# ShigemichiMatsuzaki/MSPL

Hardware: AMD Instinct MI355X
Metric: images/sec pseudo-label gen, ESPDNet-UE s=2.0 480x360(->288x480) bs=16 (higher is better)
Workload: dtype f32; 1 GPU; BASELINE configs[1]: ESPDNet-UE s=2.0 C=13 single-source pseudo-label gen (forward + pred+0.5aux argmax + KL uncertainty + histogram), bs=16/GPU, 16x3x288x480 fp32, hipGraph replay, 3 launches in flight per GPU, 2 consecutive batches of 16 per launch; per_gpu_batch=16, batches_in_flight=3, batches_per_launch=2, classes=13

## Files before the change

include/mspl_hip.h:

```cpp
#ifndef MSPL_HIP_H
#define MSPL_HIP_H

#include <stddef.h>
#include <stdint.h>

#ifdef __cplusplus
extern "C" {
#endif

typedef enum {
    MSPL_OK = 0,
    MSPL_ERR_BAD_SHAPE = -1,
    MSPL_ERR_UNSUPPORTED = -2,
    MSPL_ERR_NULL_POINTER = -3,
    MSPL_ERR_HIP = -4
} mspl_status;

typedef struct {
    const float* scale;
    const float* shift;
    const float* alpha;
    const float* pre_add;
    const float* residual;
    const float* reinf_r;
// ... 50 lines not shown
                      int32_t Wo, int32_t align_corners, const mspl_epilogue_t* ep, float* out, void* stream);

int mspl_decoder_merge_fwd(const float* enc, const float* bu, const float* w3, const float* e_scale, const float* e_shift,
                           const float* e_alpha, const float* gate, const float* b_scale, const float* b_shift,
                           const float* b_alpha, const float* wp, const float* p_scale, const float* p_shift,
                           const float* p_alpha, int32_t N, int32_t Cin, int32_t Cout, int32_t P, int32_t H, int32_t W,
                           float* out, void* stream);

int mspl_adaptive_avgpool_fwd(const float* x, int32_t N, int32_t C, int32_t Hi, int32_t Wi,
                              int32_t Ho, int32_t Wo, const mspl_epilogue_t* ep, float* out,
                              void* stream);

int mspl_pointwise_fwd(const float* x, int32_t N, int32_t C, int32_t HW, const mspl_epilogue_t* ep,
                       float* out, void* stream);

int mspl_gap_gate_fwd(const float* x, const float* w, int32_t N, int32_t Cin, int32_t Cout,
                      int32_t HW, float* mean_ws, float* gate, void* stream);

int mspl_fusion_gate_fwd(const float* z, const float* rgb, const float* depth, int64_t count, float* out, void* stream);
int mspl_fusion_gate_bwd(const float* z, const float* rgb, const float* depth, const float* gy, int64_t count,
                         float* gz, float* grgb, float* gdepth, void* stream);

int mspl_avgpool3x3s2_psum_blocks(int32_t H, int32_t W);
int mspl_avgpool3x3s2_psum_fwd(const float* x, int32_t N, int32_t C, int32_t H, int32_t W, const mspl_epilogue_t* ep, float* out,
                               float* psum, void* stream);
int mspl_gate_from_sums_fwd(const float* psum, const float* w, int32_t N, int32_t Cin, int32_t Cout, int32_t nblk, int32_t HW,
                            float* gate, void* stream);

int mspl_down_head_fits(int32_t N, int32_t nin, int32_t n, int32_t groups, int32_t H, int32_t W, uint32_t launch_flags);
int mspl_down_head_psum_blocks(int32_t H, int32_t W);
int mspl_down_head_fwd(const float* x, const float* wp, const float* pscale, const float* pshift, const float* palpha, int32_t N,
                       int32_t nin, int32_t n, int32_t groups, int32_t H, int32_t W, const mspl_epilogue_t* ep, float* r, float* out,
                       float* psum, void* stream);

int64_t mspl_pyr_down_prep_lds_bytes(int32_t N, int32_t P, int32_t h, int32_t w, int32_t nb, const int32_t* hs,
                                     const int32_t* ws);
int mspl_pyr_down_prep_fwd(const float* x, int32_t N, int32_t P, int32_t h, int32_t w, int32_t nb, const int32_t* hs,
                           const int32_t* ws, const float* const* stage_w, float* const* out, void* stream);
int mspl_pyr_down_prep_train_fwd(const float* x, int32_t N, int32_t P, int32_t h, int32_t w, int32_t nb, const int32_t* hs,
                                 const int32_t* ws, const float* const* stage_w, float* const* out, float* const* pooled,
                                 void* stream);
int mspl_pyr_down_mid_bwd(const float* const* g_e, const float* const* pooled, const float* const* stage_w, int32_t N, int32_t P,
                          int32_t h, int32_t w, int32_t nb, const int32_t* hs, const int32_t* ws, float* const* gw,
                          float* const* gx, void* stream);

int mspl_pyrpool_fused_fwd(const float* x, int32_t N, int32_t P, int32_t h, int32_t w, int32_t nb,
                           const int32_t* hs, const int32_t* ws, const float* const* stage_w,
                           const float* const* down_e, const float* br_scale, const float* br_shift,
                           const float* br_alpha, const float* merge_w, const mspl_epilogue_t* ep,
                           float* out, void* stream);

int mspl_pyrpool_fused_train_fwd(const float* x, int32_t N, int32_t P, int32_t h, int32_t w, int32_t nb,
                                 const int32_t* hs, const int32_t* ws, const float* const* stage_w,
                                 const float* const* down_e, const float* br_scale, const float* br_shift,
                                 const float* br_alpha, const float* merge_w, const mspl_epilogue_t* ep,
                                 float* out, float* zcat, void* stream);
int mspl_pyrpool_fused_train_fits(int32_t N, int32_t P, int32_t h, int32_t w, int32_t nb, const int32_t* hs, const int32_t* ws);
int mspl_pyrpool_merge_bwd(const float* gy, const float* mraw, const float* zcat, int32_t N, int32_t P, int32_t h,
                           int32_t w, int32_t nb, const float* br_scale, const float* br_shift, const float* br_alpha,
                           const float* br_mean, const float* br_inv, const float* merge_w, const float* m_scale,
                           const float* m_shift, const float* m_alpha, const float* m_mean, const float* m_inv,
                           float* gt, float* g_br_scale, float* g_br_shift, float* g_br_alpha, float* g_merge_w,
                           float* g_m_scale, float* g_m_shift, float* g_m_alpha, void* stream);
int mspl_pyrpool_branch_bwd_fits(int32_t N, int32_t P, int32_t h, int32_t w, int32_t nb, const int32_t* hs, const int32_t* ws);
int mspl_pyrpool_branch_bwd(const float* x, int32_t N, int32_t P, int32_t h, int32_t w, int32_t nb, const int32_t* hs,
                            const int32_t* ws, const float* const* stage_w, const float* const* gt, float* const* gw,
// ... 212 lines not shown
```

mspl_amd/_native.py:

```python
import ctypes
import os

import torch

_HERE = os.path.dirname(os.path.abspath(__file__))
LIB_PATH = os.environ.get('MSPL_HIP_LIB') or os.path.join(_HERE, 'lib', 'libmspl_hip.so')

c_f32p = ctypes.c_void_p
c_i32 = ctypes.c_int32
c_i64 = ctypes.c_int64


class Epilogue(ctypes.Structure):
    _fields_ = [('scale', ctypes.c_void_p), ('shift', ctypes.c_void_p), ('alpha', ctypes.c_void_p),
                ('pre_add', ctypes.c_void_p), ('residual', ctypes.c_void_p), ('reinf_r', ctypes.c_void_p),
                ('reinf_w', ctypes.c_void_p), ('gate', ctypes.c_void_p),
                ('out_ctot', c_i32), ('out_coff', c_i32), ('raw_out', ctypes.c_void_p),
                ('struct_size', ctypes.c_uint32), ('flags', ctypes.c_uint32)]


class TrainRec(ctypes.Structure):
    _fields_ = [(n, ctypes.c_void_p) for n in ('scale_x', 'scale_y', 'dscale_x', 'dscale_y', 'out_x', 'out_y', 'near_x', 'near_y',
                                               'near_out_x', 'near_out_y')] + \
               [(n, c_i32) for n in ('sh', 'sw', 'pad_h', 'pad_w', 'crop_i', 'crop_j', 'flip', 'reserved')]
# ... 5 lines not shown
ABI_VERSION = 4
ERR_UNSUPPORTED = -2
LAUNCH_THROUGHPUT = 1
LAUNCH_K2_STREAM_OFF = 2
LAUNCH_K2_STREAM_FORCE = 4


_EP = ctypes.POINTER(Epilogue)

SIGNATURES = {
    'mspl_eesp_dw_hff_fwd': [c_f32p, c_f32p, ctypes.POINTER(c_i32), c_i32, c_i32, c_i32, c_i32, c_i32, _EP,
                             c_f32p, ctypes.c_void_p],
    'mspl_eesp_proj_dw_hff_fits': [c_i32] * 6 + [ctypes.POINTER(c_i32), ctypes.c_uint32],
    'mspl_eesp_proj_dw_hff_fwd': [c_f32p] * 6 + [ctypes.POINTER(c_i32)] + [c_i32] * 6 + [_EP, c_f32p, ctypes.c_void_p],
    'mspl_eesp_dw_exp_fits': [c_i32] * 4 + [ctypes.POINTER(c_i32), ctypes.c_uint32],
    'mspl_eesp_dw_exp_pack_floats': [c_i32],
    'mspl_eesp_dw_exp_pack': [c_f32p] * 5 + [c_i32] * 3 + [ctypes.POINTER(c_i32), c_f32p, ctypes.c_void_p],
    'mspl_eesp_dw_exp_fwd': [c_f32p, c_f32p, ctypes.POINTER(c_i32)] + [c_i32] * 4 + [_EP, c_f32p, ctypes.c_void_p],
    'mspl_eesp_dw_exp_next_pack_floats': [c_i32],
    'mspl_eesp_dw_exp_next_pack': [c_f32p, c_i32, c_f32p, ctypes.c_void_p],
    'mspl_eesp_dw_exp_next_fwd': [c_f32p, c_f32p, ctypes.POINTER(c_i32)] + [c_i32] * 4 + [_EP, c_f32p] + [c_f32p] * 5 + [ctypes.c_void_p],
    'mspl_conv1x1_fwd': [c_f32p, c_f32p, c_i32, c_i32, c_i32, c_i32, c_i32, _EP, c_f32p, ctypes.c_void_p],
    'mspl_conv3x3_fwd': [c_f32p, c_f32p, c_i32, c_i32, c_i32, c_i32, c_i32, c_i32, c_i32, c_i32, _EP, c_f32p,
                         ctypes.c_void_p],
    'mspl_avgpool3x3s2_fwd': [c_f32p, c_i32, c_i32, c_i32, c_i32, _EP, c_f32p, ctypes.c_void_p],
    'mspl_bilinear_fwd': [c_f32p, c_i32, c_i32, c_i32, c_i32, c_i32, c_i32, c_i32, _EP, c_f32p, ctypes.c_void_p],
    'mspl_decoder_merge_fwd': [c_f32p] * 14 + [c_i32] * 6 + [c_f32p, ctypes.c_void_p],
    'mspl_adaptive_avgpool_fwd': [c_f32p, c_i32, c_i32, c_i32, c_i32, c_i32, c_i32, _EP, c_f32p, ctypes.c_void_p],
    'mspl_avgpool3x3s2_psum_fwd': [c_f32p, c_i32, c_i32, c_i32, c_i32, _EP, c_f32p, c_f32p, ctypes.c_void_p],
    'mspl_avgpool3x3s2_psum_blocks': [c_i32, c_i32],
    'mspl_down_head_fits': [c_i32] * 6 + [ctypes.c_uint32],
    'mspl_down_head_psum_blocks': [c_i32, c_i32],
    'mspl_down_head_fwd': [c_f32p] * 5 + [c_i32] * 6 + [_EP, c_f32p, c_f32p, c_f32p, ctypes.c_void_p],
    'mspl_gate_from_sums_fwd': [c_f32p, c_f32p, c_i32, c_i32, c_i32, c_i32, c_i32, c_f32p, ctypes.c_void_p],
    'mspl_pointwise_fwd': [c_f32p, c_i32, c_i32, c_i32, _EP, c_f32p, ctypes.c_void_p],
    'mspl_gap_gate_fwd': [c_f32p, c_f32p, c_i32, c_i32, c_i32, c_i32, c_f32p, c_f32p, ctypes.c_void_p],
    'mspl_fusion_gate_fwd': [c_f32p, c_f32p, c_f32p, c_i64, c_f32p, ctypes.c_void_p],
    'mspl_fusion_gate_bwd': [c_f32p, c_f32p, c_f32p, c_f32p, c_i64, c_f32p, c_f32p, c_f32p, ctypes.c_void_p],
    'mspl_pyrpool_fused_fwd': [c_f32p, c_i32, c_i32, c_i32, c_i32, c_i32, ctypes.POINTER(c_i32), ctypes.POINTER(c_i32),
                               ctypes.POINTER(ctypes.c_void_p), ctypes.POINTER(ctypes.c_void_p), c_f32p, c_f32p, c_f32p,
                               c_f32p, _EP, c_f32p, ctypes.c_void_p],
    'mspl_pyrpool_fused_train_fwd': [c_f32p, c_i32, c_i32, c_i32, c_i32, c_i32, ctypes.POINTER(c_i32), ctypes.POINTER(c_i32),
                                     ctypes.POINTER(ctypes.c_void_p), ctypes.POINTER(ctypes.c_void_p), c_f32p, c_f32p, c_f32p,
                                     c_f32p, _EP, c_f32p, c_f32p, ctypes.c_void_p],
    'mspl_pyrpool_fused_train_fits': [c_i32] * 5 + [ctypes.POINTER(c_i32), ctypes.POINTER(c_i32)],
    'mspl_pyrpool_merge_bwd': [c_f32p] * 3 + [c_i32] * 5 + [c_f32p] * 19 + [ctypes.c_void_p],
    'mspl_pyrpool_branch_bwd_fits': [c_i32] * 5 + [ctypes.POINTER(c_i32), ctypes.POINTER(c_i32)],
    'mspl_pyrpool_branch_bwd': [c_f32p] + [c_i32] * 5 + [ctypes.POINTER(c_i32), ctypes.POINTER(c_i32)] +
                               [ctypes.POINTER(ctypes.c_void_p)] * 3 + [c_f32p, c_f32p, c_f32p, ctypes.c_void_p],
    'mspl_label_epilogue_fwd': [c_f32p, c_f32p, c_i32, c_i32, c_i32, c_i32, c_i32, c_i32, c_i32, c_i32,
                                ctypes.c_void_p, ctypes.c_void_p, c_f32p, c_f32p, c_f32p, c_f32p, ctypes.c_void_p],
    'mspl_label_epilogue_hist_fwd': [c_f32p, c_f32p, c_i32, c_i32, c_i32, c_i32, c_i32, c_i32, c_i32, c_i32,
                                     ctypes.c_void_p, ctypes.c_void_p, c_f32p, ctypes.c_void_p, c_i32, ctypes.c_void_p, c_i64,
                                     ctypes.c_void_p],
    'mspl_label_epilogue_hist_workspace_bytes': [c_i32, c_i32, c_i32],
    'mspl_label_epilogue_hist_fits': [c_i32] * 8,
    'mspl_conv_bwd_data': [c_f32p, c_f32p] + [c_i32] * 10 + [c_f32p, ctypes.c_void_p],
    'mspl_conv_bwd_weight': [c_f32p, c_f32p] + [c_i32] * 10 + [c_f32p, ctypes.c_void_p],
    'mspl_affine_prelu_bwd': [c_f32p] * 7 + [c_i32] * 3 + [c_f32p] * 5 + [ctypes.c_void_p],
    'mspl_bn_train_small_fits': [c_i32] * 3,
    'mspl_bn_train_small_fwd': [c_f32p] * 5 + [c_i32] * 3 + [ctypes.c_float] * 2 + [c_f32p] * 2 + [ctypes.c_void_p] + [c_f32p] * 5 + [ctypes.c_void_p],
    'mspl_bn_train_small_bwd': [c_f32p] * 9 + [c_i32] * 4 + [c_f32p] * 5 + [ctypes.c_void_p],
    'mspl_bn_train_prelu_bwd_apply': [c_f32p] * 7 + [c_i32] * 3 + [c_f32p, ctypes.c_void_p],
    'mspl_pyrpool_merge_fwd': [c_f32p] + [c_i32] * 5 + [c_f32p] * 5 + [ctypes.c_void_p],
    'mspl_bn_stats_path_add': [c_f32p] * 4 + [c_i32] * 4 + [ctypes.c_void_p],
    'mspl_bn_fused_workspace_bytes': [c_i32],
# ... 64 lines not shown
                           [c_f32p] * 12 + [ctypes.c_void_p],
    'mspl_eesp_dw_bwd': [c_f32p, c_f32p, c_f32p, ctypes.POINTER(c_i32), c_i32, c_i32, c_i32, c_i32, c_i32, c_f32p,
                         ctypes.POINTER(ctypes.c_void_p), ctypes.c_void_p],
    'mspl_png_writer_create': [c_i32, c_i32],
    'mspl_png_writer_submit': [ctypes.c_void_p, ctypes.c_void_p, c_i32, c_i32, c_i32, ctypes.POINTER(ctypes.c_char_p), ctypes.c_void_p],
    'mspl_png_writer_poll': [ctypes.c_void_p, c_i64, c_i32],
    'mspl_png_writer_destroy': [ctypes.c_void_p],
    'mspl_abi_version': [],
    'mspl_sum_n': [ctypes.POINTER(ctypes.c_void_p), c_i32, c_i64, c_f32p, ctypes.c_void_p],
    'mspl_sum_n_planes': [ctypes.POINTER(ctypes.c_void_p), c_i32, c_f32p, ctypes.c_float, c_i32, c_i32, c_f32p, ctypes.c_void_p],
    'mspl_transpose_weights': [ctypes.c_void_p, ctypes.c_void_p, c_i32, ctypes.c_void_p],
    'mspl_adam_step': [c_f32p, c_f32p, c_f32p, c_f32p, c_i64, ctypes.c_float, ctypes.c_double, ctypes.c_double, ctypes.c_float, ctypes.c_float,
                       c_i32, ctypes.c_void_p],
    'mspl_merge_labels_fwd': [ctypes.POINTER(ctypes.c_void_p), c_i32, c_i64, c_i32, c_i32, c_i32, ctypes.c_void_p,
                              ctypes.c_void_p, ctypes.c_void_p],
}


def _load():
    if not os.path.isfile(LIB_PATH):
        raise ImportError(
            'mspl_amd: %s not found. Build it with `python -c "import __graft_entry__ as g; g.build()"` or '
            '`make -C mspl_amd/csrc` (hipcc --offload-arch=gfx950). There is no CPU fallback.' % LIB_PATH)
    lib = ctypes.CDLL(LIB_PATH)
    for name, argtypes in SIGNATURES.items():
        fn = getattr(lib, name)
        fn.argtypes = argtypes
        fn.restype = ctypes.c_int
    lib.mspl_pyr_down_prep_lds_bytes.restype = ctypes.c_int64
    lib.mspl_nid_workspace_floats.restype = ctypes.c_int64
    lib.mspl_eesp_dw_exp_pack_floats.restype = ctypes.c_int64
    lib.mspl_bn_fused_workspace_bytes.restype = ctypes.c_int64
    lib.mspl_eesp_dw_exp_next_pack_floats.restype = ctypes.c_int64
    lib.mspl_label_epilogue_hist_workspace_bytes.restype = ctypes.c_int64
    lib.mspl_train_transform_workspace_bytes.restype = ctypes.c_int64
    lib.mspl_png_writer_create.restype = ctypes.c_void_p
    lib.mspl_png_writer_submit.restype = ctypes.c_int64
    lib.mspl_version.restype = ctypes.c_char_p
    if lib.mspl_abi_version() != ABI_VERSION:
        raise ImportError('mspl_amd: %s has ABI revision %d, this package binds revision %d: rebuild the library (make -C mspl_amd/csrc)'
                          % (LIB_PATH, lib.mspl_abi_version(), ABI_VERSION))
    lib.mspl_last_error.argtypes = [ctypes.c_char_p, ctypes.c_size_t]
    lib.mspl_last_error.restype = ctypes.c_size_t
    return lib


lib = _load()


def last_error():
    buf = ctypes.create_string_buffer(512)
    lib.mspl_last_error(buf, 512)
    return buf.value.decode()


def check(status):
    if status != 0:
        raise RuntimeError('mspl_hip (%d): %s' % (status, last_error()))


def version():
    return lib.mspl_version().decode()
```

mspl_amd/layers.py:

```python
import math
import os
import weakref

import torch
from torch import nn

from . import autograd as ag
from . import ops
from .ops import Epi

config_inp_reinf = 3
PYR_SCALES = (2.0, 1.5, 1.0, 0.5, 0.1)


_PARAM_EPOCH = [0]


def bump_param_epoch():
    _PARAM_EPOCH[0] += 1


def _key(tensors):
    return (_PARAM_EPOCH[0],) + tuple((t.data_ptr(), t._version) for t in tensors)

# ... 102 lines not shown
    for t in outs:
        t.record_stream(cur)


def _training_path():
    return torch.is_grad_enabled()


def _conv_train(x, conv):
    if conv.kernel_size[0] == 3 and conv.dilation[0] != 1:
        raise RuntimeError('mspl_amd: dilated 3x3 convolutions only occur inside EESP (fused branch op)')
    return ag.conv(x, conv.weight, conv.stride[0], conv.groups)


def _bn_act(z, bn, alpha=None, pre_add=None, residual=None):
    if bn.training:
        if pre_add is not None:
            z, pre_add = z + pre_add, None
        if _FUSED_BN_TRAIN:
            return ag.bn_train_prelu(z, bn, alpha, residual)
        scale, shift = ag.bn_batch_stats(z, bn)
    else:
        scale, shift = train_fold(bn)
        return ag.bn_prelu(z, bn, scale, shift, alpha, pre_add=pre_add, residual=residual)
    return ag.affine_prelu(z, scale, shift, alpha, pre_add=pre_add, residual=residual)


_FUSED_TRAIN_FWD = os.environ.get('MSPL_TRAIN_FUSED_FWD', '1') != '0'
_EESP_DW_BN = os.environ.get('MSPL_EESP_DW_BN', '1') != '0'
_CONV_SKIP = os.environ.get('MSPL_CONV_SKIP', '1') != '0'
_FUSED_BN_TRAIN = os.environ.get('MSPL_FUSED_BN_TRAIN', '1') != '0'
_FUSED_DW_EXP = os.environ.get('MSPL_EESP_EXP', '1') != '0'
_FUSED_DOWN_HEAD = os.environ.get('MSPL_DOWN_HEAD', '1') != '0'
_FUSED_DEC_MERGE = True
_FUSED_NEXT_PROJ = os.environ.get('MSPL_EESP_NEXT', '1') != '0'
_FUSED_EESP_TRAIN = os.environ.get('MSPL_FUSED_EESP_TRAIN', '1') != '0'
_FUSED_PYR_TRAIN = os.environ.get('MSPL_FUSED_PYR_TRAIN', '1') != '0'


def _conv_bn_act(x, conv, bn, alpha=None, pre_add=None, residual=None):
    if bn.training or not _FUSED_TRAIN_FWD:
        return _bn_act(_conv_train(x, conv), bn, alpha, pre_add, residual)
    if conv.kernel_size[0] == 3 and conv.dilation[0] != 1:
        raise RuntimeError('mspl_amd: dilated 3x3 convolutions only occur inside EESP (fused branch op)')
    scale, shift = train_fold(bn)
    return ag.conv_bn_prelu(x, conv.weight, conv.stride[0], conv.groups, bn, scale, shift, alpha, pre_add, residual)


def train_fold(bn):
    def build():
        scale = bn.weight * ag.frozen_bn_inv(bn)
        return scale, torch.addcmul(bn.bias, bn.running_mean, scale, value=-1.0)
    return cached(bn, 'tfold', [bn.weight, bn.bias, bn.running_mean, bn.running_var], build)


def prefold_frozen_bn(model):
    bns = [m for m in model.modules() if isinstance(m, nn.BatchNorm2d) and not m.training]
    if not bns:
        return
    with torch.no_grad():
        invs = [ag.frozen_bn_inv(m) for m in bns]
        scales = torch._foreach_mul([m.weight for m in bns], invs)
        shifts = torch._foreach_addcmul([m.bias for m in bns], [m.running_mean for m in bns], scales, value=-1.0)
    for m, sc, sh in zip(bns, scales, shifts):
        store = m.__dict__.setdefault('_mspl_cache', {})
        store['tfold'] = (_key([m.weight, m.bias, m.running_mean, m.running_var]), (sc, sh))
# ... 129 lines not shown

class EESP(nn.Module):
    def __init__(self, nIn, nOut, stride=1, k=4, r_lim=7, down_method='esp'):
        super().__init__()
        self.stride = stride
        n = int(nOut / k)
        n1 = nOut - (k - 1) * n
        assert down_method in ['avg', 'esp'], 'One of these is suppported (avg or esp)'
        assert n == n1, "n(={}) and n1(={}) should be equal for Depth-wise Convolution ".format(n, n1)
        if k != 4:
            raise NotImplementedError('mspl_amd: the fused EESP kernel is built for k=4 branches')
        self.proj_1x1 = CBR(nIn, n, 1, stride=1, groups=k)
        self.dilations = eesp_dilations(r_lim, k)
        self.spp_dw = nn.ModuleList(CDilated(n, n, kSize=3, stride=stride, groups=n, d=d) for d in self.dilations)
        self.conv_1x1_exp = CB(nOut, nOut, 1, 1, groups=k)
        self.br_after_cat = BR(nOut)
        self.module_act = nn.PReLU(nOut)
        self.downAvg = True if down_method == 'avg' else False
        self.k = k

    def _dw_weights(self):
        ws = [m.conv.weight for m in self.spp_dw]
        return cached(self, 'w4', ws, lambda: torch.stack([w.reshape(-1, 3, 3) for w in ws]).contiguous())

    def _dw_exp_packed(self, H, W):
        br, exp = self.br_after_cat, self.conv_1x1_exp
        deps = [m.conv.weight for m in self.spp_dw] + [br.bn.weight, br.bn.bias, br.bn.running_mean, br.bn.running_var,
                                                      br.act.weight, exp.conv.weight]

        def build():
            bs, bb = bn_fold(br.bn)
            return ops.eesp_dw_exp_pack(self._dw_weights(), bs, bb, br.act.weight, exp.conv.weight, H, W, self.dilations)
        return cached(self, 'dwexp%dx%d' % (H, W), deps, build)

    def reduce_transform(self, input):
        scale, shift = bn_fold(self.br_after_cat.bn)
        pj = self.proj_1x1
        if ops.eesp_proj_dw_hff_fits(input.shape, pj.conv.out_channels, pj.conv.groups, self.dilations, self.stride):
            ps, pb = bn_fold(pj.bn)
            return ops.eesp_proj_dw_hff(input, pj.conv.weight, ps, pb, pj.act.weight, self._dw_weights(), self.dilations,
                                        pj.conv.groups, Epi(scale, shift, self.br_after_cat.act.weight))
        return self.transform(pj(input))

    def transform(self, o1):
        scale, shift = bn_fold(self.br_after_cat.bn)
        return ops.eesp_dw_hff(o1, self._dw_weights(), self.dilations, self.stride,
                               Epi(scale, shift, self.br_after_cat.act.weight))

    def _forward_train(self, input):
        pj, br, exp = self.proj_1x1, self.br_after_cat, self.conv_1x1_exp
        if _FUSED_EESP_TRAIN and not (pj.bn.training or br.bn.training or exp.bn.training):
            strided_avg = self.stride == 2 and self.downAvg
            residual = (not strided_avg) and self.stride == 1 and exp.conv.out_channels == input.shape[1]
            cfg = {'stride': self.stride, 'dil': tuple(self.dilations), 'groups': pj.conv.groups, 'residual': residual}
            ws = [m.conv.weight for m in self.spp_dw]
            folds = [ag.frozen_bn_fold(bn, *train_fold(bn)) for bn in (pj.bn, br.bn, exp.bn)]
            return ag.EESPFn.apply(input, cfg, *folds, pj.conv.weight, pj.bn.weight, pj.bn.bias,
                                   pj.act.weight, ws[0], ws[1], ws[2], ws[3], br.bn.weight, br.bn.bias, br.act.weight,
                                   exp.conv.weight, exp.bn.weight, exp.bn.bias, None if strided_avg else self.module_act.weight)
        has_res = self.stride == 1 and exp.conv.out_channels == input.shape[1] and not (self.stride == 2 and self.downAvg)
        skip = input
        if has_res and pj.bn.training and _CONV_SKIP and input.requires_grad:
            z1, skip = ag.conv_skip(input, pj.conv.weight, pj.conv.groups)
            o1 = _bn_act(z1, pj.bn, pj.act.weight)
        else:
            o1 = self.proj_1x1(input)
# ... 107 lines not shown
                shift = shift + rb
            return scale.contiguous(), shift.contiguous(), rw
        return cached(self, 'epi%d' % int(with_reinf), deps, build)

    def _forward_train(self, input, input2, alias=None):
        avg_out = ag.avgpool(input)
        eesp_out = self.eesp(input if alias is None else alias)
        reinf = None
        if input2 is not None:
            with torch.no_grad():
                pyr = input2 if isinstance(input2, ImagePyramid) else ImagePyramid(input2)
                img = pyr.at_height(avg_out.shape[2])
            if img.shape[3] != avg_out.shape[3]:
                raise RuntimeError('The size of tensor a (%d) must match the size of tensor b (%d) at non-singleton '
                                   'dimension 3' % (avg_out.shape[3], img.shape[3]))
            reinf = self.inp_reinf(img)
        return ag.down_tail(avg_out, eesp_out, self.act.weight, reinf)

    def forward(self, input, input2=None, _alias=None):
        if _training_path():
            return self._forward_train(input, input2, _alias)
        N, _, H, W = input.shape
        Ho, Wo = (H - 1) // 2 + 1, (W - 1) // 2 + 1
        out = torch.empty((N, self.nout, Ho, Wo), device=input.device, dtype=torch.float32)
        r = None
        if input2 is not None:
            pyr = input2 if isinstance(input2, ImagePyramid) else ImagePyramid(input2)
            with fork(0, (pyr.levels[0],)):
                r = self.inp_reinf[0](pyr.at_height(Ho))
            if r.shape[3] != Wo:
                raise RuntimeError('The size of tensor a (%d) must match the size of tensor b (%d) at non-singleton '
                                   'dimension 3' % (Wo, r.shape[3]))
        pj = self.eesp.proj_1x1
        if _FUSED_DOWN_HEAD and ops.down_head_fits(input.shape, pj.conv.out_channels, pj.conv.groups):
            join(0, (r,))
            scale, shift, rw = self._epilogue_vectors(r is not None)
            ep = Epi(scale, shift, self.act.weight, reinf_r=r, reinf_w=rw)
            ps, pb = bn_fold(pj.bn)
            o1, sums = ops.down_head(input, pj.conv.weight, ps, pb, pj.act.weight, pj.conv.groups, ep, out)
            _remember_plane_sums(input, sums)
            cat = self.eesp.transform(o1)
            ops.conv1x1(cat, self.eesp.conv_1x1_exp.conv.weight, self.eesp.k, ep, out=(out, self.nin))
            return out
        cat = self.eesp.reduce_transform(input)
        join(0, (r,))
        scale, shift, rw = self._epilogue_vectors(r is not None)
        ep = Epi(scale, shift, self.act.weight, reinf_r=r, reinf_w=rw)
        _, sums = ops.avgpool3x3s2(input, ep, out=(out, 0), plane_sums=True)
        _remember_plane_sums(input, sums)
        ops.conv1x1(cat, self.eesp.conv_1x1_exp.conv.weight, self.eesp.k, ep, out=(out, self.nin))
        return out


_PLANE_SUMS = weakref.WeakKeyDictionary()


class _TensorKey(object):
    __slots__ = ('__weakref__',)


def _remember_plane_sums(t, sums):
    key = getattr(t, '_mspl_key', None)
    if key is None:
        key = _TensorKey()
        t._mspl_key = key
    _PLANE_SUMS[key] = (t.data_ptr(), t._version, sums)


def _recall_plane_sums(t):
    key = getattr(t, '_mspl_key', None)
    hit = _PLANE_SUMS.get(key) if key is not None else None
    if hit is None or hit[0] != t.data_ptr() or hit[1] != t._version:
        return None
    return hit[2]

# ... 204 lines not shown
```

mspl_amd/ops.py:

```python
import ctypes
import math

import torch

from . import _native as nat
from ._native import Epilogue, check, lib


def _stream():
    return ctypes.c_void_p(torch.cuda.current_stream().cuda_stream)


def _f32(t, name):
    if not isinstance(t, torch.Tensor) or not t.is_cuda:
        raise RuntimeError('mspl_amd: %s must be a CUDA (ROCm) tensor; there is no CPU path' % name)
    if t.dtype != torch.float32:
        raise RuntimeError('mspl_amd: %s must be float32, got %s' % (name, t.dtype))
    if not t.is_contiguous():
        t = t.contiguous()
    return t


def _p(t):
    return None if t is None else ctypes.c_void_p(t.data_ptr())
# ... 233 lines not shown
        return dst
    nblk = lib.mspl_avgpool3x3s2_psum_blocks(H, W)
    if nblk <= 0:
        check(nblk)
    sums = torch.empty((N * C, nblk), device=x.device, dtype=torch.float32)
    check(lib.mspl_avgpool3x3s2_psum_fwd(_p(x), N, C, H, W, ctypes.byref(s), _p(dst), _p(sums), _stream()))
    return dst, sums


def down_head_fits(shape, n, groups):
    N, nin, H, W = [int(v) for v in shape]
    return bool(lib.mspl_down_head_fits(N, nin, int(n), int(groups), H, W, current_launch_flags()))


def down_head(x, wproj, pscale, pshift, palpha, groups, ep, out):
    x, wproj = _f32(x, 'x'), _f32(wproj, 'projection weight')
    N, nin, H, W = x.shape
    n = wproj.shape[0]
    if wproj.numel() != n * (nin // groups) or nin % groups or n % groups:
        raise RuntimeError('mspl_amd: down_head weight %s does not match nin=%d groups=%d' % (tuple(wproj.shape), nin, groups))
    ps, pb, pa = _vec(pscale, n, 'pscale'), _vec(pshift, n, 'pshift'), _vec(palpha, n, 'palpha')
    dst, coff = _dest((out, 0), (N, nin, H // 2, W // 2), x)
    s, keep = _build(ep, dst, coff, N, nin, (H // 2) * (W // 2))
    nblk = lib.mspl_down_head_psum_blocks(H, W)
    if nblk <= 0:
        check(nblk)
    r = torch.empty((N, n, H, W), device=x.device, dtype=torch.float32)
    sums = torch.empty((N * nin, nblk), device=x.device, dtype=torch.float32)
    check(lib.mspl_down_head_fwd(_p(x), _p(wproj), _p(ps), _p(pb), _p(pa), N, nin, n, int(groups), H, W, ctypes.byref(s), _p(r),
                                 _p(dst), _p(sums), _stream()))
    return r, sums


def gate_from_sums(plane_sums, w, hw):
    w = _f32(w, 'w')
    Cout = w.shape[0]
    Cin = w.numel() // Cout
    planes, nblk = plane_sums.shape
    N = planes // Cin
    if planes != N * Cin or plane_sums.dtype != torch.float32 or not plane_sums.is_contiguous():
        raise RuntimeError('mspl_amd: gate_from_sums: sums %s do not match Cin=%d' % (tuple(plane_sums.shape), Cin))
    gate = torch.empty((N, Cout), device=w.device, dtype=torch.float32)
    check(lib.mspl_gate_from_sums_fwd(_p(plane_sums), _p(w), N, Cin, Cout, nblk, int(hw), _p(gate), _stream()))
    return gate


def decoder_merge_shape_ok(Cin, Cout, P, H, W):
    groups = math.gcd(Cin, Cout)
    cg, cob = Cin // groups, Cout // groups
    if H % 2 or W % 2 or H < 2 or W < 2 or P not in (2, 6, 10, 16) or Cout > 1024:
        return False
    return (cg, cob) in ((1, 1), (8, 3)) or ((cg, cob) == (4, 1) and groups >= 16 and W % 4 == 0 and 16 <= W <= 256 and H >= 4)


def decoder_merge(enc, bu, w3, e_epi, gate, b_epi, wp, p_epi):
    enc, bu, w3, wp = _f32(enc, 'enc'), _f32(bu, 'bu'), _f32(w3, 'w3'), _f32(wp, 'wp')
    N, Cin, H, W = enc.shape
    Cout, P = w3.shape[0], wp.shape[0]
    if tuple(bu.shape) != (N, Cout, H // 2, W // 2) or H % 2 or W % 2:
        return None
    groups = math.gcd(Cin, Cout)
    if tuple(w3.shape) != (Cout, Cin // groups, 3, 3) or wp.numel() != P * Cout:
        raise RuntimeError('mspl_amd: decoder_merge weights %s / %s do not match Cin=%d Cout=%d'
                           % (tuple(w3.shape), tuple(wp.shape), Cin, Cout))
    gate = _vec(gate, N * Cout, 'gate')
    es, eb, ea = [_vec(t, Cout, 'expansion epilogue') for t in e_epi]
# ... 228 lines not shown
```

Baseline: 21390 images/s.

## Fuse strided dilated depthwise, HFF, BN-PReLU and grouped 1x1 expansion in downsampling EESP

Adds a HIP kernel for the strided EESP downsampling block. It computes the four stride-2 dilated depthwise branches with hierarchical feature fusion and BN+PReLU in LDS, then runs the grouped 1x1 expansion on MFMA 32x32x2 f32. The outer epilogue with reinforcement is applied directly into the concatenated output. This removes the intermediate concat tensor round-trip and separate launches, in exchange for a shape-specialised path (n=32, W=120, dilations 1-4) plus a packed-weight cache.

```diff
diff --git a/include/mspl_hip.h b/include/mspl_hip.h
--- a/include/mspl_hip.h
+++ b/include/mspl_hip.h
@@ -106,6 +106,13 @@
 int mspl_down_head_fwd(const float* x, const float* wp, const float* pscale, const float* pshift, const float* palpha, int32_t N,
                        int32_t nin, int32_t n, int32_t groups, int32_t H, int32_t W, const mspl_epilogue_t* ep, float* r, float* out,
                        float* psum, void* stream);
+
+int mspl_down_dw_exp_fits(int32_t N, int32_t n, int32_t H, int32_t W, const int32_t dil[4], uint32_t launch_flags);
+int64_t mspl_down_dw_exp_pack_floats(int32_t n);
+int mspl_down_dw_exp_pack(const float* w4, const float* bscale, const float* bshift, const float* balpha, const float* wexp,
+                          int32_t n, float* packed, void* stream);
+int mspl_down_dw_exp_fwd(const float* r, const float* packed, const int32_t dil[4], int32_t N, int32_t n, int32_t H, int32_t W,
+                         const mspl_epilogue_t* ep, float* out, void* stream);
 
 int64_t mspl_pyr_down_prep_lds_bytes(int32_t N, int32_t P, int32_t h, int32_t w, int32_t nb, const int32_t* hs,
                                      const int32_t* ws);
diff --git a/mspl_amd/_native.py b/mspl_amd/_native.py
--- a/mspl_amd/_native.py
+++ b/mspl_amd/_native.py
@@ -61,6 +61,10 @@
     'mspl_down_head_fits': [c_i32] * 6 + [ctypes.c_uint32],
     'mspl_down_head_psum_blocks': [c_i32, c_i32],
     'mspl_down_head_fwd': [c_f32p] * 5 + [c_i32] * 6 + [_EP, c_f32p, c_f32p, c_f32p, ctypes.c_void_p],
+    'mspl_down_dw_exp_fits': [c_i32] * 4 + [ctypes.POINTER(c_i32), ctypes.c_uint32],
+    'mspl_down_dw_exp_pack_floats': [c_i32],
+    'mspl_down_dw_exp_pack': [c_f32p] * 5 + [c_i32, c_f32p, ctypes.c_void_p],
+    'mspl_down_dw_exp_fwd': [c_f32p, c_f32p, ctypes.POINTER(c_i32)] + [c_i32] * 4 + [_EP, c_f32p, ctypes.c_void_p],
     'mspl_gate_from_sums_fwd': [c_f32p, c_f32p, c_i32, c_i32, c_i32, c_i32, c_i32, c_f32p, ctypes.c_void_p],
     'mspl_pointwise_fwd': [c_f32p, c_i32, c_i32, c_i32, _EP, c_f32p, ctypes.c_void_p],
     'mspl_gap_gate_fwd': [c_f32p, c_f32p, c_i32, c_i32, c_i32, c_i32, c_f32p, c_f32p, ctypes.c_void_p],
@@ -191,6 +195,7 @@
     lib.mspl_eesp_dw_exp_pack_floats.restype = ctypes.c_int64
     lib.mspl_bn_fused_workspace_bytes.restype = ctypes.c_int64
     lib.mspl_eesp_dw_exp_next_pack_floats.restype = ctypes.c_int64
+    lib.mspl_down_dw_exp_pack_floats.restype = ctypes.c_int64
     lib.mspl_label_epilogue_hist_workspace_bytes.restype = ctypes.c_int64
     lib.mspl_train_transform_workspace_bytes.restype = ctypes.c_int64
     lib.mspl_png_writer_create.restype = ctypes.c_void_p
diff --git a/mspl_amd/csrc/down_dw_exp.hip b/mspl_amd/csrc/down_dw_exp.hip
--- /dev/null
+++ b/mspl_amd/csrc/down_dw_exp.hip
@@ -0,0 +1,303 @@
+#include <stdlib.h>
+
+#include "common.hpp"
+
+namespace mspl {
+
+typedef float dx_f32x16 __attribute__((ext_vector_type(16)));
+
+constexpr int DX_REC = 48;
+constexpr int DX_MAXD = 4;
+
+__device__ __forceinline__ int dx_xcd_remap(int bid, int nwg) {
+    const int q = nwg >> 3, r = nwg & 7, xcd = bid & 7;
+    const int base = (xcd < r) ? xcd * (q + 1) : r * (q + 1) + (xcd - r) * q;
+    return base + (bid >> 3);
+}
+
+__global__ void down_dw_exp_pack_kernel(const float* __restrict__ w4, const float* __restrict__ bscale, const float* __restrict__ bshift,
+                                        const float* __restrict__ balpha, const float* __restrict__ wexp, int n,
+                                        float* __restrict__ dwp, float* __restrict__ ap) {
+    const int i = blockIdx.x * blockDim.x + threadIdx.x;
+    if (i < n * DX_REC) {
+        const int c = i / DX_REC, f = i - c * DX_REC;
+        const int k = f / 12, e = f - k * 12;
+        float v;
+        if (e < 9) v = w4[((size_t)k * n + c) * 9 + e];
+        else if (e == 9) v = bscale[k * n + c];
+        else if (e == 10) v = bshift[k * n + c];
+        else v = balpha[k * n + c];
+        dwp[i] = v;
+    }
+    const int hk = n / 2;
+    if (i < 4 * 64 * hk) {
+        const int lane = i & 63, s = (i >> 6) % hk, g = i / (hk * 64);
+        const int m = lane & 31, k = 2 * s + (lane >> 5);
+        ap[i] = m < n ? wexp[(size_t)(g * n + m) * n + k] : 0.f;
+    }
+}
+
+template <int NCH, int WO, int TH, int KC>
+__global__ __launch_bounds__(512, 4) void down_dw_exp_kernel(const float* __restrict__ r, const float* __restrict__ dwp,
+                                                             const float* __restrict__ ap, Epi e, float* __restrict__ out,
+                                                             int H, int bands, int nwg) {
+    constexpr int MAXD = DX_MAXD;
+    constexpr int ROWS = 2 * TH - 1 + 2 * MAXD;
+    constexpr int PH = 2;
+    constexpr int HS = WO + 2 * PH;
+    constexpr int RS = 2 * HS;
+    constexpr int PX = TH * WO;
+    constexpr int NS64 = (PX + 63) / 64;
+    constexpr int SPW = NS64 / 2;
+    constexpr int SLOTS = NS64 * 64;
+    constexpr int NCHUNK = NCH / KC;
+    constexpr int LPR = WO <= 64 ? 64 : 128;
+    constexpr int RPP = 512 / LPR;
+    constexpr int IPT = (KC * ROWS + RPP - 1) / RPP;
+    static_assert(WO <= 128, "staging: one float2 column per thread");
+    constexpr int TPW = KC * NS64 / 8;
+    static_assert(NS64 % 2 == 0 && (KC * NS64) % 8 == 0, "eight waves: (group, half of the sub-tiles) / (channel, sub-tile)");
+    static_assert(KC % 2 == 0 && NCH % KC == 0 && NCHUNK >= 2 && NCH % 8 == 0 && NCH <= 32, "chunking");
+    static_assert(WO % 2 == 0, "8-byte stores: pixel pairs never straddle a row");
+
+    constexpr int RT_F = KC * ROWS * RS, BB_F = 4 * KC * SLOTS;
+    static_assert((2 * RT_F + 2 * BB_F) * 4 <= 64 * 1024, "static LDS");
+    __shared__ __attribute__((aligned(16))) float lds_[2 * RT_F + 2 * BB_F];
+    float* const rt_[2] = {lds_, lds_ + RT_F};
+    float* const bb_[2] = {lds_ + 2 * RT_F, lds_ + 2 * RT_F + BB_F};
+
+    const int tid = threadIdx.x;
+    const int lane = tid & 63;
+    const int wave = __builtin_amdgcn_readfirstlane(tid >> 6);
+    const int li = lane & 31, half = lane >> 5;
+
+    const int lid = dx_xcd_remap(blockIdx.x, nwg);
+    const int band = lid % bands;
+    const int img = lid / bands;
+    const int y0 = band * TH;
+    const int Ho = H >> 1;
+    const int HWi = H * 2 * WO;
+
+    const float* rimg = r + (size_t)img * NCH * HWi;
+    const int c2 = tid % LPR, r0 = tid / LPR;
+    const bool cok = c2 < WO;
+    float2 sv[IPT];
+    auto load_chunk = [&](int c) {
+        const float* rc = rimg + (size_t)c * KC * HWi + 2 * (cok ? c2 : 0);
+#pragma unroll
+        for (int q = 0; q < IPT; ++q) {
+            const int fr = r0 + RPP * q;
+            const int j = fr / ROWS, row = fr - j * ROWS;
+            const int gy = 2 * y0 - MAXD + row;
+            const bool ok = cok && fr < KC * ROWS && gy >= 0 && gy < H;
+            const float2 v = *reinterpret_cast<const float2*>(rc + (ok ? j * HWi + gy * (2 * WO) : 0));
+            sv[q] = ok ? v : make_float2(0.f, 0.f);
+        }
+    };
+    auto store_chunk = [&](float* dst) {
+        float* d = dst + r0 * RS + PH + c2;
+#pragma unroll
+        for (int q = 0; q < IPT; ++q) {
+            if (cok && r0 + RPP * q < KC * ROWS) {
+                d[RPP * q * RS] = sv[q].x;
+                d[RPP * q * RS + HS] = sv[q].y;
+            }
+        }
+    };
+
+    auto dw_stage = [&](int c, const float* src, float* dst) {
+#pragma unroll
+        for (int u = 0; u < TPW; ++u) {
+            const int task = wave + 8 * u;
+            const int j = task % KC, st = task / KC;
+            const float* rec = dwp + (size_t)(c * KC + j) * DX_REC;
+            float wv[DX_REC];
+#pragma unroll
+            for (int i = 0; i < DX_REC; ++i) wv[i] = rec[i];
+            const int p = 64 * st + lane;
+            const int pc = p < PX ? p : PX - 1;
+            const int ty = (TH > 1) ? pc / WO : 0;
+            const int tx = pc - ty * WO;
+            const float* tp = src + j * (ROWS * RS) + (2 * ty + MAXD) * RS + PH + tx;
+            float prev = 0.f;
+            float tap[4][9];
+#pragma unroll
+            for (int k = 0; k < 4; ++k) {
+                const int d = k + 1;
+#pragma unroll
+                for (int ky = 0; ky < 3; ++ky)
+#pragma unroll
+                    for (int kx = 0; kx < 3; ++kx) {
+                        const int q = ky * 3 + kx;
+                        const int o = (kx - 1) * d;
+                        const int col = (o & 1) ? HS + (o - 1) / 2 : o / 2;
+                        if (q == 4 && k > 0) tap[k][q] = tap[0][4];
+                        else tap[k][q] = tp[(ky - 1) * d * RS + col];
+                    }
+                float a = 0.f;
+#pragma unroll
+                for (int ky = 0; ky < 3; ++ky) {
+                    a = fmaf(wv[k * 12 + ky * 3 + 0], tap[k][ky * 3 + 0], a);
+                    a = fmaf(wv[k * 12 + ky * 3 + 1], tap[k][ky * 3 + 1], a);
+                    a = fmaf(wv[k * 12 + ky * 3 + 2], tap[k][ky * 3 + 2], a);
+                }
+                a += prev;
+                prev = a;
+                float q = fmaf(a, wv[k * 12 + 9], wv[k * 12 + 10]);
+                q = q > 0.f ? q : wv[k * 12 + 11] * q;
+                dst[(k * KC + j) * SLOTS + p] = q;
+            }
+        }
+    };
+
+    const int g = wave & 3, sh = wave >> 2;
+    dx_f32x16 acc[SPW][2];
+#pragma unroll
+    for (int u = 0; u < SPW; ++u)
+#pragma unroll
+        for (int i = 0; i < 16; ++i) { acc[u][0][i] = 0.f; acc[u][1][i] = 0.f; }
+    const float* apw = ap + (size_t)g * (NCH / 2) * 64 + lane;
+    float a_cur[KC / 2], a_nxt[KC / 2];
+    auto load_a = [&](int c, float (&dst)[KC / 2]) {
+#pragma unroll
+        for (int i = 0; i < KC / 2; ++i) dst[i] = apw[(c * (KC / 2) + i) * 64];
+    };
+    auto mm_stage = [&](const float* src, const float (&av)[KC / 2]) {
+#pragma unroll
+        for (int u = 0; u < SPW; ++u) {
+            const float* bp = src + (g * KC + half) * SLOTS + 64 * (sh * SPW + u) + 2 * li;
+#pragma unroll
+            for (int i = 0; i < KC / 2; ++i) {
+                const float2 b2 = *reinterpret_cast<const float2*>(bp + 2 * i * SLOTS);
+                acc[u][0] = __builtin_amdgcn_mfma_f32_32x32x2f32(av[i], b2.x, acc[u][0], 0, 0, 0);
+                acc[u][1] = __builtin_amdgcn_mfma_f32_32x32x2f32(av[i], b2.y, acc[u][1], 0, 0, 0);
+            }
+        }
+    };
+
+    load_chunk(0);
+    load_a(0, a_cur);
+    for (int i = tid; i < 2 * KC * ROWS * 8; i += 512) {
+        const int c8 = i & 7, k4 = c8 & 3;
+        const int rr = i >> 3;
+        lds_[rr * RS + (c8 >> 2) * HS + (k4 < 2 ? k4 : WO + k4)] = 0.f;
+    }
+    store_chunk(rt_[0]);
+    load_chunk(1);
+    __syncthreads();
+    dw_stage(0, rt_[0], bb_[0]);
+    store_chunk(rt_[1]);
+    __syncthreads();
+
+#pragma unroll
+    for (int c = 0; c < NCHUNK; ++c) {
+        if (c + 2 < NCHUNK) load_chunk(c + 2);
+        if (c + 1 < NCHUNK) {
+            if ((c & 1) == 0) load_a(c + 1, a_nxt); else load_a(c + 1, a_cur);
+            dw_stage(c + 1, rt_[(c + 1) & 1], bb_[(c + 1) & 1]);
+        }
+        if ((c & 1) == 0) mm_stage(bb_[c & 1], a_cur); else mm_stage(bb_[c & 1], a_nxt);
+        if (c + 2 < NCHUNK) store_chunk(rt_[c & 1]);
+        if (c + 1 < NCHUNK) __syncthreads();
+    }
+
+    const int rows_here = (Ho - y0) < TH ? (Ho - y0) : TH;
+    const int npx = rows_here * WO;
+#pragma unroll
+    for (int u = 0; u < SPW; ++u) {
+        const int p = 64 * (sh * SPW + u) + 2 * li;
+        const bool pok = p < npx;
+        const int pix = y0 * WO + (pok ? p : 0);
+        float2 r0 = make_float2(0.f, 0.f), r1 = r0, r2 = r0;
+        if (e.reinf_r) {
+            const float* rp = e.reinf_r + (size_t)img * 3 * e.hw + pix;
+            r0 = *reinterpret_cast<const float2*>(rp);
+            r1 = *reinterpret_cast<const float2*>(rp + e.hw);
+            r2 = *reinterpret_cast<const float2*>(rp + 2 * (size_t)e.hw);
+        }
+#pragma unroll
+        for (int rg = 0; rg < 4; ++rg) {
+            if (8 * rg + 8 > NCH) continue;
+#pragma unroll
+            for (int q = 0; q < 4; ++q) {
+                const int rr = rg * 4 + q;
+                const int cabs = e.coff + g * NCH + 8 * rg + 4 * half + q;
+                const EpiCh ch = epi_channel(e, cabs);
+                float v0 = fmaf(acc[u][0][rr], ch.scale, ch.shift);
+                float v1 = fmaf(acc[u][1][rr], ch.scale, ch.shift);
+                if (e.reinf_r) {
+                    v0 += ch.rw0 * r0.x + ch.rw1 * r1.x + ch.rw2 * r2.x;
+                    v1 += ch.rw0 * r0.y + ch.rw1 * r1.y + ch.rw2 * r2.y;
+                }
+                v0 = v0 > 0.f ? v0 : ch.alpha * v0;
+                v1 = v1 > 0.f ? v1 : ch.alpha * v1;
+                if (pok) store_out2(out + epi_offset(e, img, cabs, pix), make_float2(v0, v1));
+            }
+            asm volatile("" ::: "memory");
+        }
+    }
+}
+
+static int dx_plan(int n, int H, int W, const int32_t* dil) {
+    if (!dil || H < 2 || (H & 1)) return 0;
+    if (!(dil[0] == 1 && dil[1] == 2 && dil[2] == 3 && dil[3] == 4)) return 0;
+    if (n == 32 && W == 120) return 2;
+    return 0;
+}
+
+}
+
+using namespace mspl;
+
+extern "C" int mspl_down_dw_exp_fits(int32_t N, int32_t n, int32_t H, int32_t W, const int32_t dil[4], uint32_t flags) {
+    static const int enabled = MSPL_TUNE_INT("MSPL_DOWN_DW_EXP", 1);
+    (void)flags;
+    if (!enabled || N < 1) return 0;
+    return dx_plan(n, H, W, dil) != 0 ? 1 : 0;
+}
+
+extern "C" int64_t mspl_down_dw_exp_pack_floats(int32_t n) { return (int64_t)n * DX_REC + 4ll * 64 * (n / 2); }
+
+extern "C" int mspl_down_dw_exp_pack(const float* w4, const float* bscale, const float* bshift, const float* balpha,
+                                     const float* wexp, int32_t n, float* packed, void* stream_) {
+    hipStream_t stream = static_cast<hipStream_t>(stream_);
+    MSPL_REQUIRE(w4 && bscale && bshift && balpha && wexp && packed, MSPL_ERR_NULL_POINTER, "down_dw_exp_pack: null pointer");
+    MSPL_REQUIRE(n == 32, MSPL_ERR_UNSUPPORTED, "down_dw_exp_pack: n=%d not covered", n);
+    const int total = 4 * 64 * (n / 2);
+    hipLaunchKernelGGL(down_dw_exp_pack_kernel, dim3((unsigned)ceil_div(total, 256)), dim3(256), 0, stream, w4, bscale, bshift, balpha,
+                       wexp, n, packed, packed + (size_t)n * DX_REC);
+    MSPL_CHECK_LAUNCH("down_dw_exp_pack");
+    return MSPL_OK;
+}
+
+extern "C" int mspl_down_dw_exp_fwd(const float* r, const float* packed, const int32_t dil[4], int32_t N, int32_t n, int32_t H,
+                                    int32_t W, const mspl_epilogue_t* ep, float* out, void* stream_) {
+    hipStream_t stream = static_cast<hipStream_t>(stream_);
+    MSPL_REQUIRE(r && packed && dil && ep && out, MSPL_ERR_NULL_POINTER, "down_dw_exp: null pointer");
+    MSPL_REQUIRE(N >= 1 && H >= 1 && W >= 1, MSPL_ERR_BAD_SHAPE, "down_dw_exp: N=%d H=%d W=%d", N, H, W);
+    if (int rc = check_epi(ep, 4 * n, "down_dw_exp")) return rc;
+    MSPL_REQUIRE(ep->scale && ep->shift && ep->alpha, MSPL_ERR_NULL_POINTER, "down_dw_exp: the block's epilogue needs scale, shift and alpha");
+    MSPL_REQUIRE(!ep->pre_add && !ep->residual && !ep->gate && !ep->raw_out, MSPL_ERR_UNSUPPORTED,
+                 "down_dw_exp: only scale/shift/alpha and the reinforcement");
+    const int kind = dx_plan(n, H, W, dil);
+    MSPL_REQUIRE(kind != 0, MSPL_ERR_UNSUPPORTED, "down_dw_exp: n=%d H=%d W=%d dil=%d,%d,%d,%d not covered", n, H, W, dil[0], dil[1], dil[2],
+                 dil[3]);
+    MSPL_REQUIRE((((uintptr_t)r | (uintptr_t)out | (uintptr_t)packed | (uintptr_t)ep->reinf_r) & 15) == 0, MSPL_ERR_BAD_SHAPE,
+                 "down_dw_exp: operands must be 16-byte aligned");
+    const int Ho = H / 2, Wo = W / 2;
+    const Epi e = make_epi(ep, 4 * n, Ho * Wo);
+    MSPL_REQUIRE((int64_t)N * n * H * W < (1ll << 31) && (int64_t)N * e.ctot * Ho * Wo < (1ll << 31), MSPL_ERR_BAD_SHAPE,
+                 "down_dw_exp: tensor too large");
+    constexpr int TH = 2;
+    const int bands = ceil_div(Ho, TH);
+    const int64_t nwg = (int64_t)N * bands;
+    MSPL_REQUIRE(nwg < (1ll << 30), MSPL_ERR_BAD_SHAPE, "down_dw_exp: grid too large");
+    const float* dwp = packed;
+    const float* ap = packed + (size_t)n * DX_REC;
+    const dim3 grid((unsigned)nwg), blk(512);
+#define DX_ARGS grid, blk, 0, stream, r, dwp, ap, e, out, H, bands, (int)nwg
+    hipLaunchKernelGGL((down_dw_exp_kernel<32, 60, TH, 4>), DX_ARGS);
+#undef DX_ARGS
+    MSPL_CHECK_LAUNCH("down_dw_exp");
+    return MSPL_OK;
+}
diff --git a/mspl_amd/layers.py b/mspl_amd/layers.py
--- a/mspl_amd/layers.py
+++ b/mspl_amd/layers.py
@@ -158,6 +158,7 @@
 _FUSED_BN_TRAIN = os.environ.get('MSPL_FUSED_BN_TRAIN', '1') != '0'
 _FUSED_DW_EXP = os.environ.get('MSPL_EESP_EXP', '1') != '0'
 _FUSED_DOWN_HEAD = os.environ.get('MSPL_DOWN_HEAD', '1') != '0'
+_FUSED_DOWN_DW_EXP = os.environ.get('MSPL_DOWN_DW_EXP', '1') != '0'
 _FUSED_DEC_MERGE = True
 _FUSED_NEXT_PROJ = os.environ.get('MSPL_EESP_NEXT', '1') != '0'
 _FUSED_EESP_TRAIN = os.environ.get('MSPL_FUSED_EESP_TRAIN', '1') != '0'
@@ -353,6 +354,16 @@
             bs, bb = bn_fold(br.bn)
             return ops.eesp_dw_exp_pack(self._dw_weights(), bs, bb, br.act.weight, exp.conv.weight, H, W, self.dilations)
         return cached(self, 'dwexp%dx%d' % (H, W), deps, build)
+
+    def _down_dw_exp_packed(self):
+        br, exp = self.br_after_cat, self.conv_1x1_exp
+        deps = [m.conv.weight for m in self.spp_dw] + [br.bn.weight, br.bn.bias, br.bn.running_mean, br.bn.running_var,
+                                                      br.act.weight, exp.conv.weight]
+
+        def build():
+            bs, bb = bn_fold(br.bn)
+            return ops.down_dw_exp_pack(self._dw_weights(), bs, bb, br.act.weight, exp.conv.weight)
+        return cached(self, 'downdwexp', deps, build)
 
     def reduce_transform(self, input):
         scale, shift = bn_fold(self.br_after_cat.bn)
@@ -526,6 +537,8 @@
                 raise RuntimeError('The size of tensor a (%d) must match the size of tensor b (%d) at non-singleton '
                                    'dimension 3' % (Wo, r.shape[3]))
         pj = self.eesp.proj_1x1
+        tail = _FUSED_DOWN_DW_EXP and self.eesp.conv_1x1_exp.conv.groups == 4 \
+            and ops.down_dw_exp_fits((N, pj.conv.out_channels, H, W), self.eesp.dilations)
         if _FUSED_DOWN_HEAD and ops.down_head_fits(input.shape, pj.conv.out_channels, pj.conv.groups):
             join(0, (r,))
             scale, shift, rw = self._epilogue_vectors(r is not None)
@@ -533,8 +546,20 @@
             ps, pb = bn_fold(pj.bn)
             o1, sums = ops.down_head(input, pj.conv.weight, ps, pb, pj.act.weight, pj.conv.groups, ep, out)
             _remember_plane_sums(input, sums)
+            if tail:
+                ops.down_dw_exp(o1, self.eesp._down_dw_exp_packed(), self.eesp.dilations, ep, out=(out, self.nin))
+                return out
             cat = self.eesp.transform(o1)
             ops.conv1x1(cat, self.eesp.conv_1x1_exp.conv.weight, self.eesp.k, ep, out=(out, self.nin))
+            return out
+        if tail:
+            o1 = pj(input)
+            join(0, (r,))
+            scale, shift, rw = self._epilogue_vectors(r is not None)
+            ep = Epi(scale, shift, self.act.weight, reinf_r=r, reinf_w=rw)
+            _, sums = ops.avgpool3x3s2(input, ep, out=(out, 0), plane_sums=True)
+            _remember_plane_sums(input, sums)
+            ops.down_dw_exp(o1, self.eesp._down_dw_exp_packed(), self.eesp.dilations, ep, out=(out, self.nin))
             return out
         cat = self.eesp.reduce_transform(input)
         join(0, (r,))
diff --git a/mspl_amd/ops.py b/mspl_amd/ops.py
--- a/mspl_amd/ops.py
+++ b/mspl_amd/ops.py
@@ -289,6 +289,35 @@
     return r, sums
 
 
+def down_dw_exp_fits(shape, dilations):
+    N, n, H, W = [int(v) for v in shape]
+    d = (ctypes.c_int32 * 4)(*[int(v) for v in dilations])
+    return bool(lib.mspl_down_dw_exp_fits(N, n, H, W, d, current_launch_flags()))
+
+
+def down_dw_exp_pack(w4, bscale, bshift, balpha, wexp):
+    w4 = _f32(w4, 'w4')
+    n = w4.shape[1]
+    if tuple(w4.shape) != (4, n, 3, 3):
+        raise RuntimeError('mspl_amd: down_dw_exp weight %s, expected (4,%d,3,3)' % (tuple(w4.shape), n))
+    bs, bb, ba = _vec(bscale, 4 * n, 'bscale'), _vec(bshift, 4 * n, 'bshift'), _vec(balpha, 4 * n, 'balpha')
+    wexp = _vec(wexp, 4 * n * n, 'expansion weight')
+    packed = torch.empty(int(lib.mspl_down_dw_exp_pack_floats(n)), device=w4.device, dtype=torch.float32)
+    check(lib.mspl_down_dw_exp_pack(_p(w4), _p(bs), _p(bb), _p(ba), _p(wexp), n, _p(packed), _stream()))
+    return packed
+
+
+def down_dw_exp(r, packed, dilations, ep, out):
+    r = _f32(r, 'r')
+    N, n, H, W = r.shape
+    packed = _vec(packed, int(lib.mspl_down_dw_exp_pack_floats(n)), 'packed')
+    dst, coff = _dest(out, (N, 4 * n, H // 2, W // 2), r)
+    s, keep = _build(ep, dst, coff, N, 4 * n, (H // 2) * (W // 2))
+    d = (ctypes.c_int32 * 4)(*[int(v) for v in dilations])
+    check(lib.mspl_down_dw_exp_fwd(_p(r), _p(packed), d, N, n, H, W, ctypes.byref(s), _p(dst), _stream()))
+    return dst
+
+
 def gate_from_sums(plane_sums, w, hw):
     w = _f32(w, 'w')
     Cout = w.shape[0]
```

After: 21430 images/s (median of 6 runs). Within noise of the previous version (+0.2%).
